# KAS-W/Deep-Reinforcement-Learning-Based-Signal-Gated-Market-Making

Hardware: AMD Instinct MI355X
Metric: env-steps/sec (pop×ticks) at 1/2/4/8 MI355X; generations/sec vs CPU ref (higher is better)
Workload: dtype f32+f64; 1 GPU; BASELINE config 3: 5 GA population(s) x 512 individuals (phi=0.0001 tick=0.001 510300, phi=0.001 tick=0.001 510300, phi=0.005 tick=0.001 510300, phi=0.008 tick=0.001 510300, phi=0.01 tick=0.001 510300), TradingPolicy 3->32->32->2, synthetic ticks (4560 train + 912 validation: the new master of each population), 1 GPU(s), weak scaling; config_id=3, populations=5, population_global=512, population_per_gpu=512, hidden=32, ticks_train=4560, ticks_val=912, adversary=False, val_mode=best, parallelism=population shards x1, hip_graph=True, walk_feedback=True

## Files before the change

deep-reinforcement-learning-based-signal-gated-market-making_amd/csrc/sgmm_frontier.hip:

```cpp
#include <cstddef>
#include <cstdlib>
#include <cstring>

#include "sgmm_mlp_mfma.h"

namespace sgmm {

#ifdef SGMM_STAMPS
constexpr int kStampWaves = 1 << 16;
__device__ unsigned long long g_tstamps[kStampWaves][8];
__device__ unsigned int g_thwid[kStampWaves][2];
#endif

struct FusedChain {
    double S;
    uint32_t st;
    int32_t tr;
};
template <class T>
__device__ __forceinline__ T fused_ld(const T* p) {
    typedef __attribute__((address_space(1))) const T gT;
    return __hip_atomic_load((gT*)p, __ATOMIC_RELAXED, __HIP_MEMORY_SCOPE_AGENT);
}
template <class T>
__device__ __forceinline__ void fused_st(T* p, T v) {
    typedef __attribute__((address_space(1))) T gT;
    __hip_atomic_store((gT*)p, v, __ATOMIC_RELAXED, __HIP_MEMORY_SCOPE_AGENT);
}

__device__ __forceinline__ FusedChain fused_group(const FrontierArgs& args, int e, int g, int CL, int nch,
                                                  FusedChain cs, double* win, uint32_t* kin, uint8_t* start) {
    const EpArrays& ep = args.ep;
    const int lane = (int)threadIdx.x;
    const int32_t T = ep.len[e];
    const int c0 = g * kFrontierLanes, c1 = min(nch, c0 + kFrontierLanes);
// ... 150 lines not shown
    if (ng > 1 && cg == 1) {
        if (threadIdx.x == 0) go = __hip_atomic_load(hs, __ATOMIC_RELAXED, __HIP_MEMORY_SCOPE_AGENT) == 1u;
        if (!__shfl(go, 0, kWave)) {
            fused_ship(args, e, CL, nch);
            if (threadIdx.x == 0) {
                asm volatile("s_waitcnt vmcnt(0)" ::: "memory");
                go = __hip_atomic_fetch_add(hs, 2u, __ATOMIC_RELAXED, __HIP_MEMORY_SCOPE_AGENT) == 1u;
            }
            if (!__shfl(go, 0, kWave)) return;
        }
        const double S0 = fused_ld(&ho->S);
        const uint32_t w = fused_ld(&ho->st_tr);
        cs = FusedChain{S0, w & 0xFFu, (int32_t)(w >> 8)};
        g = 1;
    }
    asm volatile("s_waitcnt vmcnt(0)" ::: "memory");
    for (;;) {
        cs = fused_group(args, e, g, CL, nch, cs, win, kin, start);
        if (g + 1 >= ng) break;
        go = 0;
        if (threadIdx.x == 0) {
            fused_st(&ho->S, cs.S);
            fused_st(&ho->st_tr, cs.st | ((uint32_t)cs.tr << 8));
            asm volatile("s_waitcnt vmcnt(0)" ::: "memory");
            go = __hip_atomic_fetch_add(hs, 1u, __ATOMIC_RELAXED, __HIP_MEMORY_SCOPE_AGENT) == 2u;
        }
        if (!__shfl(go, 0, kWave)) return;
        g = 1;
    }
    if (ng > 1 && threadIdx.x == 0) fused_st(hs, 0u);
    fused_finish(args, e, cs);
}

template <int H, int NSI, int LS, bool SP, bool FS = false>
__global__ __launch_bounds__(kWave) __attribute__((amdgpu_waves_per_eu(4))) void k_policy_frontier(FrontierArgs args) {
    static_assert(!FS || (LS == 1 && !SP), "the fused scan: one wave per walk, no spill");
    static_assert(H % 16 == 0 && H <= 32, "frontier kernel: H = 16 or 32");
    using L = GenomeLayout<H>;
    constexpr int NT = H / 16, KS = H / 4;
    constexpr int HP = 20;
    constexpr int kHb = kWave * HP * 4;
    constexpr int kBig = L::N * 4 > kHb ? L::N * 4 : kHb;
    __shared__ __attribute__((aligned(16))) unsigned char big[kBig];
    __shared__ __attribute__((aligned(16))) float w3i[2 * H + 2];
    __shared__ __attribute__((aligned(16))) float c1s[NT][4][4];
    __shared__ __attribute__((aligned(16))) float b2s[H];
    __shared__ __attribute__((aligned(8))) float sig[kWave][2];
    __shared__ double px[5][kWave];
    __shared__ uint16_t pl[kWave * (NSI - 1)];
    __shared__ uint32_t nslot_s;
    __shared__ uint32_t wid_s, tmin_s, t0_s, spk_s;
    constexpr int kFa0 = (int)(offsetof(FrontierArgs, ep) / 4), kFa1 = (int)(offsetof(FrontierArgs, src) / 4);
    constexpr int kFa2 = (int)(offsetof(FrontierArgs, inv_min) / 4), kFa3 = (int)(sizeof(FrontierArgs) / 4);
    constexpr int kFaWords = (kFa1 - kFa0) + (kFa3 - kFa2);
    static_assert(offsetof(FrontierArgs, src) % 4 == 0 && offsetof(FrontierArgs, inv_min) % 4 == 0 &&
                  sizeof(FrontierArgs) % 4 == 0, "whole words");
    __shared__ uint32_t fa_s[FS ? kFaWords : 1];
    __shared__ uint32_t ep_s, cl_s, nch_s, cg_s;
#if defined(__HIP_DEVICE_COMPILE__)
    if constexpr (FS) {
        typedef __attribute__((address_space(4))) const uint32_t ka_u32;
        const ka_u32* ka = (const ka_u32*)__builtin_amdgcn_kernarg_segment_ptr();
        for (int i = (int)threadIdx.x; i < kFaWords; i += kWave)
            fa_s[i] = ka[i < kFa1 - kFa0 ? kFa0 + i : kFa2 + i - (kFa1 - kFa0)];
    }
#endif
    if (SP && threadIdx.x == 0) {
        wid_s = blockIdx.x;
        spk_s = 0;
        t0_s = (uint32_t)wall_clock64();
        args.wspill[blockIdx.x] = 0u;
    }

    const sgmm_ticks& tk = args.tk;
    const EpArrays& ep = args.ep;
    const sgmm_env_params* __restrict__ params = args.params;
    const GenomeSrc& src = args.src;
    const int32_t inv_min = args.inv_min, nsi = args.nsi;
    uint64_t* __restrict__ cmaps = args.cmaps;
    uint32_t* __restrict__ ctr32 = args.ctr32;
    uint32_t* __restrict__ kinfo = args.kinfo;
    double* __restrict__ rew = args.rew;
    static_assert(LS == 1 || LS == 2 || LS == 4, "lane split 1, 2 or 4");
    constexpr int NL = kFrontierLanes / LS;
    int pos, cg, nw;
    frontier_wave(ep, (int)blockIdx.x / LS, pos, cg, nw);
    const int off = ((int)blockIdx.x % LS) * NL;
    const int e = ep.order ? ep.order[pos] : pos;
    const int32_t T = ep.len[e];
    if (T <= 0) {
        if (!FS || cg != 0) return;
        if (threadIdx.x == 0) {
            ep_s = (uint32_t)e;
            cl_s = 4u;
            nch_s = 0u;
            cg_s = 0u;
        }
    }
    if (T > 0) {
        const int CL = frontier_len(T, nw);
        const int nch = (T + CL - 1) / CL;
        if (cg * kFrontierLanes + off >= nch) return;
        if (FS && threadIdx.x == 0) {
            ep_s = (uint32_t)e;
            cl_s = (uint32_t)CL;
            nch_s = (uint32_t)nch;
            cg_s = (uint32_t)cg;
// ... 8 lines not shown

        float* gsm = reinterpret_cast<float*>(big);
        stage_genomes(src, e, ep.genome[e], -1, L::N, gsm, nullptr);
        __syncthreads();
        if (lane < 2 * H) w3i[lane] = gsm[L::W3 + (lane & 1) * H + (lane >> 1)];
        if (lane < 2) w3i[2 * H + lane] = gsm[L::B3 + lane];
        if (lane < H) {
            b2s[lane] = gsm[L::B2 + lane];
            c1s[lane >> 4][lane & 3][(lane >> 2) & 3] = gsm[L::B1 + lane];
        }
        float a1[NT];
#pragma unroll
        for (int hf = 0; hf < NT; ++hf)
            a1[hf] = grp < 3 ? gsm[L::W1 + 3 * (16 * hf + 4 * (col & 3) + (col >> 2)) + grp] : 0.0f;
        float w2f[NT][KS];
#pragma unroll
        for (int rt = 0; rt < NT; ++rt)
#pragma unroll
            for (int i = 0; i < KS; ++i) w2f[rt][i] = gsm[L::W2 + (16 * rt + col) * H + 4 * i + grp];
        __syncthreads();
        float* hb = reinterpret_cast<float*>(big);
        const sgmm_env_params p = params[ep.param[e]];

        const uint32_t all = (1u << nsi) - 1u;
        const uint32_t sset = (!lane_ok || c >= nch) ? 0u : (c == 0 ? 1u << (uint32_t)(-inv_min) : all);
        const uint32_t p0 = sset ? (uint32_t)__builtin_ctz(sset) : 0u;
        uint64_t cur = kIdentityMap;
        uint32_t cnt[(NSI + 1) / 2];
#pragma unroll
        for (int s = 0; s < (NSI + 1) / 2; ++s) cnt[s] = 0;
        uint32_t mcnt = 0;
        bool merged = __builtin_popcount(sset) <= 1;
        int kc = merged ? 0 : CL;
        auto tick_of = [&](int tt) { return tb + (ntl > 0 ? t0 : 0) + min(tt, max(ntl - 1, 0)); };
#ifdef SGMM_STAMPS
        unsigned long long lite_t0, lite_sl = 0, lite_ts = 0, lite_s8 = 0, lite_s16 = 0;
        asm volatile("s_memrealtime %0\n\ts_waitcnt lgkmcnt(0)" : "=s"(lite_t0)::"memory");
#endif
#ifdef SGMM_STAMPS_PHASE
        unsigned long long fs_t0, fs_a, fs_b, fs_c[7] = {0, 0, 0, 0, 0, 0, 0}, fs_r0;
#define SGMM_FT(var) asm volatile("s_memtime %0\n\ts_waitcnt lgkmcnt(0)" : "=s"(var)::"memory")
        asm volatile("s_memrealtime %0\n\ts_waitcnt lgkmcnt(0)" : "=s"(fs_r0)::"memory");
        SGMM_FT(fs_t0);
#define SGMM_PH(k)                    \
        do {                              \
            unsigned long long t_;        \
            SGMM_FT(t_);                  \
            fs_c[k] += t_ - fs_b;         \
            fs_b = t_;                    \
        } while (0)
#else
#define SGMM_PH(k) \
        do {           \
        } while (0)
#endif
        int64_t ti = tick_of(0);
        float ns1 = tk.s1n[ti], ns2 = tk.s2n[ti];
        int fr_extra = 0;
        if ((SP || LS == 1) && lane == 0) {
            nslot_s = 0;
            if (SP) tmin_s = (uint32_t)max(4, CL - kSpillTicks);
        }

        auto mlp = [&](auto nq, float& o0, float& o1, auto&& after_layer2) {
            constexpr int NQ = decltype(nq)::value;
            float xb[NQ];
#pragma unroll
            for (int q = 0; q < NQ; ++q) xb[q] = hb[(16 * q + col) * 4 + grp];
            f32x4 acc[NQ][NT];
#pragma unroll
            for (int q0 = 0; q0 < NQ; q0 += 2) {
                constexpr int Q2 = NQ < 2 ? NQ : 2;
                f32x4 h1[Q2][NT];
#pragma unroll
                for (int hf = 0; hf < NT; ++hf) {
                    const f32x4 cc = *reinterpret_cast<const f32x4*>(&c1s[hf][grp][0]);
#pragma unroll
                    for (int q = 0; q < Q2; ++q)
                        h1[q][hf] = __builtin_amdgcn_mfma_f32_16x16x4f32(a1[hf], xb[q0 + q], cc, 0, 0, 0);
                }
#pragma unroll
                for (int q = 0; q < Q2; ++q)
#pragma unroll
                    for (int hf = 0; hf < NT; ++hf)
#pragma unroll
                        for (int r = 0; r < 4; ++r) h1[q][hf][r] = relu(h1[q][hf][r]);
#pragma unroll
                for (int rt = 0; rt < NT; ++rt) {
                    const f32x4 bb = *reinterpret_cast<const f32x4*>(&b2s[16 * rt + 4 * grp]);
#pragma unroll
// ... 28 lines not shown
                    asm volatile("" : "+v"(w3p));
                    const f32x4 h = *reinterpret_cast<const f32x4*>(&hb[lane * HP + 4 * j4]);
#pragma unroll
                    for (int r2 = 0; r2 < 2; ++r2) {
                        const f32x4 w = *reinterpret_cast<lds_cf4*>(w3p + 4 * r2);
                        o0 = __builtin_fmaf(w[0], h[2 * r2], o0);
                        o1 = __builtin_fmaf(w[1], h[2 * r2], o1);
                        o0 = __builtin_fmaf(w[2], h[2 * r2 + 1], o0);
                        o1 = __builtin_fmaf(w[3], h[2 * r2 + 1], o1);
                    }
                }
                asm volatile("" ::: "memory");
            }
#ifdef SGMM_STAMPS_PHASE
            asm volatile("s_waitcnt vmcnt(0) lgkmcnt(0)" ::: "memory");
#endif
            SGMM_PH(2);
        };

#pragma unroll 1
        for (int tt = 0; tt < CL; ++tt) {
#ifdef SGMM_STAMPS_PHASE
            SGMM_FT(fs_b);
#endif
            if constexpr (SP) {
                if ((tt & 3) == 0 && (uint32_t)tt >= (uint32_t)__builtin_amdgcn_readfirstlane((int)tmin_s) &&
                    (uint32_t)wall_clock64() - (uint32_t)__builtin_amdgcn_readfirstlane((int)t0_s) > args.spill_budget) {
                    if (lane == 0) spk_s = (uint32_t)tt;
                    break;
                }
            }
            const bool act = tt < ntl;
            const float s1 = ns1, s2 = ns2;
            const int64_t tcur = ti;
            ti = tick_of(tt + 1);
            ns1 = tk.s1n[ti];
            ns2 = tk.s2n[ti];
            uint32_t fmask = 0;
            if (merged) {
                fmask = 1u << map_get(cur, p0);
            } else {
#pragma unroll
                for (int s = 0; s < NSI; ++s)
                    if ((sset >> s) & 1u) fmask |= 1u << map_get(cur, (uint32_t)s);
            }
            if (!act) fmask = 0;
            const uint32_t ext = fmask & (fmask - 1u);
            int epfx = 0, etot = 0;
            if (__ballot(ext != 0u)) {
                *reinterpret_cast<f32x2*>(&sig[lane][0]) = f32x2{s1, s2};
                const uint32_t nex = (uint32_t)__builtin_popcount(ext);
                const uint64_t eb0 = __ballot(nex & 1u), eb1 = __ballot(nex & 2u), eb2 = __ballot(nex & 4u);
                epfx = mbcnt64(eb0) + 2 * mbcnt64(eb1) + 4 * mbcnt64(eb2);
                etot = __popcll(eb0) + 2 * __popcll(eb1) + 4 * __popcll(eb2);
                uint32_t r = ext;
                int pp = epfx;
#pragma unroll
                for (int m = 0; m < NSI - 1; ++m)
                    if (r) {
                        pl[pp++] = (uint16_t)((lane << 3) | __builtin_ctz(r));
                        r &= r - 1u;
                    }
            }
            const bool any0 = __ballot(fmask != 0u) != 0ull;
            const int nx = (etot + kWave - 1) / kWave;
            fr_extra = fr_extra - (fr_extra >> 3) + (nx << 5);
            if ((SP || LS == 1) && lane == 0)
                __hip_atomic_fetch_add(&nslot_s, (uint32_t)((any0 ? 1 : 0) + nx), __ATOMIC_RELAXED, __HIP_MEMORY_SCOPE_WAVEFRONT);
            if ((tt & 7) == 7) {
                if (fr_extra > kFrPrioExtra) __builtin_amdgcn_s_setprio(2);
                else __builtin_amdgcn_s_setprio(0);
            }
#ifdef SGMM_STAMPS
            lite_sl += (any0 ? 1 : 0) + nx;
            if (tt == 7) lite_s8 = lite_sl;
            if (tt == 15) lite_s16 = lite_sl;
            lite_ts += (any0 ? 4 : 0) + (etot + 15) / 16;
#endif
            int64_t prs = ep.rs;
            asm volatile("" : "+s"(prs));
            const uint64_t pa = reinterpret_cast<uint64_t>(rew + rbase);
            uint64_t pu = ((uint64_t)(uint32_t)__builtin_amdgcn_readfirstlane((int)(uint32_t)(pa >> 32)) << 32) |
                          (uint32_t)__builtin_amdgcn_readfirstlane((int)(uint32_t)pa);
            asm volatile("" : "+s"(pu));
            double* const prow = reinterpret_cast<double*>(pu) + frontier_row(tt, off);
            uint64_t stepmap = kIdentityMap;
            uint32_t trm = 0;
#ifdef SGMM_STAMPS_PHASE
            fs_c[3] += (any0 ? 1 : 0) + nx;
            asm volatile("s_waitcnt vmcnt(0) lgkmcnt(0)" ::: "memory");
#endif
            SGMM_PH(5);
            if (any0) {
                const bool has = fmask != 0u;
                const uint32_t f = has ? (uint32_t)__builtin_ctz(fmask) : 0u;
                *reinterpret_cast<f32x4*>(&hb[lane * 4]) = f32x4{s1, s2, (float)(inv_min + (int)f) * 0.5f, 0.0f};
                float o0, o1;
                double tmid, task, tbid, tbmax, tsmin;
                mlp(IntC<NL / 16>{}, o0, o1, [&] {
                    tmid = tk.mid_next[tcur];
                    task = tk.best_ask[tcur];
                    tbid = tk.best_bid[tcur];
                    tbmax = tk.buy_max[tcur];
                    tsmin = tk.sell_min[tcur];
                });
                if (etot) {
                    px[0][lane] = tmid;
                    px[1][lane] = task;
                    px[2][lane] = tbid;
                    px[3][lane] = tbmax;
                    px[4][lane] = tsmin;
                }
                const int32_t oa = act_to_int(rintf(o0 * p.act_scale));
                const int32_t ob = act_to_int(rintf(o1 * p.act_scale));
                const StepOut so1 = ftp_step(p, inv_min + (int)f, oa, ob, tmid, task, tbid, tbmax, tsmin);
                if (has) {
                    const uint64_t to = (uint64_t)(f + so1.fill_buy - so1.fill_sell);
                    stepmap = (stepmap & ~(0xFFull << (8 * f))) | (to << (8 * f));
                    trm |= (uint32_t)(so1.fill_buy | so1.fill_sell) << f;
                    if (merged) {
                        prow[p0 * prs + lane] = so1.reward;
                    } else {
#pragma unroll
                        for (int s = 0; s < NSI; ++s)
                            if (((sset >> s) & 1u) && map_get(cur, (uint32_t)s) == f) prow[s * prs + lane] = so1.reward;
                    }
                }
#ifdef SGMM_STAMPS_PHASE
                asm volatile("s_waitcnt vmcnt(0) lgkmcnt(0)" ::: "memory");
#endif
                SGMM_PH(4);
            }
#pragma unroll 1
            for (int x = 0; x < nx; ++x) {
                const int pidx = kWave * x + lane;
                const bool has = pidx < etot;
                const uint32_t v = has ? (uint32_t)pl[pidx] : 0u;
// ... 277 lines not shown
                        const uint32_t ki = args.kinfo[ci];
                        const bool merged = (int)(ki & kKinfoTick) < CL;
                        const uint32_t p0 = ki >> 29;
                        const uint32_t all = (1u << nsi) - 1u;
                        const uint32_t sset = c == 0 ? 1u << (uint32_t)(-inv_min) : all;
                        const int sh = (lane >> shs) << shs;
                        const uint64_t segm = SEG == 64 ? ~0ull : (((1ull << SEG) - 1ull) << sh);
                        const int ntl = has ? min(T, (c + 1) * CL) - c * CL : 0;
                        const bool last = valid && u == ntl - K - 1;
                        uint64_t cm = cur;
#pragma unroll
                        for (int st = 0; st < NSI; ++st) {
                            const bool tr = st < nsi && ((sset >> st) & 1u);
                            const uint32_t x = map_get(cur, (uint32_t)st);
                            const uint32_t y = map_get(excl, x & 7u);
                            if (valid && tr && (!merged || (uint32_t)st == p0))
                                args.rew[(int64_t)st * ep.rs + rbase + frontier_row(K + u, lg)] = rl_s[y & 7u][lane];
                            const uint32_t cnt = (uint32_t)__popcll(__ballot(valid && tr && ((traded >> (y & 7u)) & 1u)) & segm);
                            if (last && tr) {
                                args.ctr32[ci * 8 + st] += cnt;
                                cm = (cm & ~(0xFFull << (8 * st))) | ((uint64_t)map_get(inc, x & 7u) << (8 * st));
                            }
                        }
                        if (last) args.cmaps[ci] = cm;
                    }
                    __syncthreads();
                }
            }
            __syncthreads();
        }
    }
}

int launch_frontier_spill(int hidden, int nsi, unsigned n_waves, int ls, hipStream_t s, const FrontierArgs& fa) {
    if (!fa.spill_budget || !fa.wspill || n_waves == 0) return SGMM_OK;
    const int total = (int)(n_waves * (unsigned)ls);
    const dim3 grid(kSpillBlocks), block(kWave * nsi);
    with_int<16, 32>(hidden, [&](auto h) {
        with_int<5, 8>(nsi <= 5 ? 5 : 8, [&](auto n) {
            SGMM_LAUNCH((k_frontier_spill<decltype(h)::value, decltype(n)::value>), grid, block, 0, s, fa, total, ls);
        });
    });
    SGMM_LAUNCHED();
    return SGMM_OK;
}

int launch_policy_frontier(int hidden, int nsi, unsigned n_waves, int ls, hipStream_t s, const FrontierArgs& fa) {
    const dim3 grid(n_waves), block(kWave);
    if (fa.fitness && (ls != 1 || fa.ep.ngrp > kFusedMaxGroups || fa.spill_budget || !fa.handoff || !fa.hstate)) {
        set_error("fused path scan: one wave per walk, <= %d groups, no spill, hand-off arrays", kFusedMaxGroups);
        return SGMM_ERR_ARG;
    }
    with_int<16, 32>(hidden, [&](auto h) {
        with_int<5, 8>(nsi <= 5 ? 5 : 8, [&](auto n) {
            constexpr int H = decltype(h)::value, NSI = decltype(n)::value;
            if (fa.fitness) {
                SGMM_LAUNCH((k_policy_frontier<H, NSI, 1, false, true>), grid, block, 0, s, fa);
                return;
            }
            with_bool(fa.spill_budget && fa.wspill, [&](auto sp) {
                with_int<4, 2, 1>(ls, [&](auto l) {
                    SGMM_LAUNCH((k_policy_frontier<H, NSI, decltype(l)::value, decltype(sp)::value>),
                                dim3(n_waves * (unsigned)ls), block, 0, s, fa);
                });
            });
        });
// ... 16 lines not shown
```

deep-reinforcement-learning-based-signal-gated-market-making_amd/csrc/sgmm_plan.h:

```cpp
#pragma once

#include <algorithm>
#include <cstddef>
#include <cstdint>

#include "../../include/sgmm.h"

#if defined(__HIPCC__)
#define SGMM_PLAN_HD __host__ __device__ __forceinline__
#else
#define SGMM_PLAN_HD inline
#endif

namespace sgmm {

constexpr int kWave = 64;
constexpr int kChunk = 64;
constexpr int kScanBlock = 256;
constexpr int kMaxLen = 1 << 17;
constexpr int kFrontierLanes = 64;
constexpr int kFrontierMaxWaves = 16;
constexpr int64_t kFrontierMaxLen = (int64_t)kFrontierLanes * 65532;
constexpr int kFusedMaxGroups = 2;
constexpr int kFusedHandoffBytes = 16;
constexpr int kScanThreads = 1024;
constexpr int kScanAt1024 = 256;
constexpr int kScanAt512 = 512;
constexpr int kScanArlAt1024 = 1024;
#ifndef SGMM_LANES_W
#define SGMM_LANES_W 4
#endif
constexpr int kLanesW = SGMM_LANES_W;
constexpr int kReorderMaxPops = 64;

SGMM_PLAN_HD int frontier_len(int T, int nw) {
    const int c = (T + kFrontierLanes * nw - 1) / (kFrontierLanes * nw);
    return c < 4 ? 4 : (c + 3) & ~3;
}
SGMM_PLAN_HD int64_t frontier_pad(int nw) { return 256LL * nw + 16; }

struct PlanKnobs {
    int32_t policy_path = -1;
    int32_t groups = -1;
    int32_t lane_split = -1;
    int32_t tail = -1;
    int32_t four = -1;
    int32_t min_eps = -1;
    int32_t table_sp = -1;
    int32_t scan_threads = -1;
    int32_t reorder_weights = -1;
    int32_t spill = -1;
    int32_t seq_sum = -1;
    int32_t fused_scan = -1;
    int32_t lanes_scan = -1;
};
static_assert(sizeof(PlanKnobs) == SGMM_PLAN_N * sizeof(int32_t), "one field per SGMM_PLAN_* knob");

struct LaunchShape {
    int32_t n = 0;
    int32_t max_len = 0;
    int64_t total_steps = 0;
    int32_t nsi = 0;
    int32_t hidden = 0;
    bool arl = false;
    int32_t simds = 0;
    bool tail = false;
    int32_t mode = 0;
    int32_t pop_eps = 0;
    int32_t src_pop_eps = 0;
    bool walk_feedback = false;
};

constexpr size_t kNoSection = ~size_t(0);
struct WorkspaceLayout {
    size_t cmaps = kNoSection, ctr = kNoSection, kinfo = kNoSection, wslots = kNoSection, wspill = kNoSection,
           arrive = kNoSection, handoff = kNoSection, fills = kNoSection, rew = kNoSection;
    int64_t rs = 0;
    size_t bytes = 0;
};

struct FrontierPlan {
    int32_t g0, gtail, whole, gmax;
    int64_t waves;
    int32_t ls;
};

enum class PolicyKernel { Frontier, TableSp, TableV3, TableMfma, TableValu };
enum class ScanKernel { Fused, Lanes, Wave, Arl };

struct LaunchPlan {
    PolicyKernel policy;
    FrontierPlan fr;
    uint32_t spill;
    ScanKernel scan;
    int32_t scan_threads;
    int32_t scan_grid;
    int32_t seq_sum;
    int32_t lanes_w;
    bool validation;
    bool reorder;
    uint32_t w_whole, w_split;
    WorkspaceLayout ws;
};

constexpr int kFrontierAutoWaves = 8;
inline FrontierPlan frontier_plan(int32_t n, int32_t simds, const PlanKnobs& k) {
    FrontierPlan p{1, 1, std::max(n, 0), 1, std::max<int64_t>(n, 0), 1};
    const int ls_force = k.lane_split;
    if (ls_force == 2 || ls_force == 4) p.ls = ls_force;
    {
        const int g = k.groups;
// ... 17 lines not shown
    } else if (tail && four && p.g0 == 1 && 2 * n - 4 * S >= S / 2 && n < 4 * S) {
        p.whole = (int32_t)(2 * n - 4 * S);
        p.gtail = p.gmax = 2;
    } else if (tail && p.g0 == 1 && n > S && r > 0) {
        const int64_t gt = std::max<int64_t>(1, std::min<int64_t>(kFrontierMaxWaves, (S + r / 2) / r));
        if (gt > 1) {
            p.whole = (int32_t)(n - r);
            p.gtail = p.gmax = (int32_t)gt;
        }
    }
    p.waves = (int64_t)p.whole * p.g0 + (int64_t)(n - p.whole) * p.gtail;
    return p;
}

inline int64_t plane_stride(int64_t steps, int32_t n, bool arl, int32_t gmax) {
    const int64_t pad = arl ? 0 : frontier_pad(gmax) * n;
    return (steps + pad + 31) & ~int64_t(31);
}

inline WorkspaceLayout workspace_layout(int32_t n, int64_t total_steps, int32_t nsi, bool arl, int32_t gmax) {
    WorkspaceLayout L;
    L.rs = plane_stride(total_steps, n, arl, gmax);
    if (total_steps < 0 || nsi <= 0 || nsi > 8 || n < 0) return L;
    size_t at = 0;
    const auto section = [&at](size_t bytes) {
        const size_t off = at;
        at += (bytes + 255) & ~size_t(255);
        return off;
    };
    const size_t steps = (size_t)total_steps, ne = (size_t)n;
    if (arl) {
        L.fills = section(steps * sizeof(uint64_t));
        L.rew = at;
        L.bytes = at + (size_t)L.rs * (size_t)(4 * nsi) * sizeof(double);
        return L;
    }
    const size_t slots = steps / kChunk + ne + 1;
    const size_t recs = ne * kFrontierLanes * (size_t)gmax;
    L.cmaps = section(std::max(slots, recs) * sizeof(uint64_t));
    L.ctr = section(std::max(slots * sizeof(uint64_t), recs * 8 * sizeof(uint32_t)));
    L.kinfo = section(recs * sizeof(uint32_t));
    L.wslots = section(ne * 64 * sizeof(uint32_t));
    L.wspill = section(ne * 64 * sizeof(uint32_t));
    L.arrive = section(ne * sizeof(uint32_t));
    L.handoff = section(ne * kFusedHandoffBytes);
    L.rew = at;
    L.bytes = at + (size_t)L.rs * (size_t)nsi * sizeof(double);
    return L;
}
inline WorkspaceLayout workspace_layout(int32_t n, int64_t total_steps, int32_t nsi, bool arl, int32_t simds,
                                        const PlanKnobs& k) {
    return workspace_layout(n, total_steps, nsi, arl, frontier_plan(n, simds, k).gmax);
}

constexpr int kFrontierMinEps = 512;
constexpr int64_t kTableSpChunks = 256;
inline PolicyKernel policy_kernel(const LaunchShape& sh, const PlanKnobs& k) {
    const bool h1632 = sh.hidden == 16 || sh.hidden == 32;
    const int path = k.policy_path;
    if (!sh.arl && h1632) {
        if (sh.max_len > kMaxLen || path == 1) return PolicyKernel::Frontier;
        if (path <= 0 && sh.n >= (k.min_eps > 0 ? k.min_eps : kFrontierMinEps)) return PolicyKernel::Frontier;
    }
    if (sh.hidden == 8 || path == 3) return PolicyKernel::TableValu;
    if (sh.arl || !h1632) return PolicyKernel::TableMfma;
    const int64_t nch = (sh.max_len + kChunk - 1) / kChunk;
    const bool sp = k.table_sp >= 0 ? k.table_sp != 0 : nch * sh.n <= kTableSpChunks;
    return sp ? PolicyKernel::TableSp : PolicyKernel::TableV3;
}

inline LaunchPlan resolve_plan(const LaunchShape& sh, const PlanKnobs& k) {
    LaunchPlan p{};
    p.policy = policy_kernel(sh, k);
    p.fr = frontier_plan(sh.n, sh.simds, k);
    p.ws = workspace_layout(sh.n, sh.total_steps, sh.nsi, sh.arl, p.fr.gmax);
    const bool fr = p.policy == PolicyKernel::Frontier;
    p.validation = sh.tail && (sh.mode == 2 || sh.mode == 4);
    const bool plain_tail = !sh.tail || sh.mode == 3;

    if (fr && k.spill > 0 && sh.max_len > 0) p.spill = (uint32_t)std::min<int64_t>((int64_t)k.spill * 100, 0x7FFFFFFF);

    const int P = sh.src_pop_eps;
    p.reorder = fr && sh.tail && sh.mode == 3 && sh.walk_feedback && P > 0 && sh.n % P == 0 && sh.n / P >= 2 &&
                sh.n / P <= kReorderMaxPops && p.fr.ls == 1 && p.fr.g0 == 1 && (p.fr.gtail == 2 || p.fr.gtail == 4) &&
                p.fr.whole > 0 && p.fr.whole < sh.n && sh.total_steps == (int64_t)sh.n * sh.max_len;
    p.w_whole = 5;
    p.w_split = 4;
    if (const int w = k.reorder_weights; w > 0 && (w >> 8) > 0 && (w & 255) > 0) {
        p.w_whole = (uint32_t)(w >> 8) & 63u;
        p.w_split = (uint32_t)w & 63u;
    }

    if (fr && sh.max_len > 0 && k.fused_scan != 0 && !p.validation && !p.spill && p.fr.ls == 1 &&
        p.fr.gmax <= kFusedMaxGroups && k.seq_sum != 0 && plain_tail && (k.fused_scan == 1 || p.fr.gmax == 1)) {
        p.scan = ScanKernel::Fused;
        return p;
    }

    const auto seq_sum = [&](int nt) {
        if (k.seq_sum >= 0) return k.seq_sum != 0;
        return p.validation || (!sh.arl && nt <= 256);
    };
    p.scan_grid = sh.n;
    if (sh.arl) {
        p.scan = ScanKernel::Arl;
        p.scan_threads = sh.n <= kScanArlAt1024 ? kScanThreads : kScanBlock;
        p.seq_sum = seq_sum(p.scan_threads);
        return p;
// ... 23 lines not shown
```

deep-reinforcement-learning-based-signal-gated-market-making_amd/csrc/sgmm_rollout.h:

```cpp
#pragma once

#include "sgmm_device.h"
#include "sgmm_ga_device.h"
#include "sgmm_internal.h"
#include "sgmm_plan.h"

namespace sgmm {

constexpr int kSeg = 4096;

struct EpArrays {
    const int32_t* genome;
    const int32_t* adv;
    const int64_t* tick_off;
    const int32_t* len;
    const int64_t* step_off;
    const int32_t* param;
    int64_t rs;
    const int32_t* order;
    int32_t ngrp;
    int32_t g0, gtail, whole;
    int32_t seq_sum = 0;
};

// ... 120 lines not shown
    }
}
constexpr uint32_t kKinfoTick = 0xFFFFu;
__host__ __device__ __forceinline__ uint32_t kinfo_groups(uint32_t k) { return (k >> 20) & 31u; }

struct StepArgs {
    sgmm_ga_state* st;
    float* master_mm;
    float* master_adv;
    float* best_master;
    int64_t n_mm, n_adv;
    uint64_t seed;
    sgmm_ga_history* history;
    int32_t hist_cap;
    int32_t P;
    int32_t pop_eps;
    const uint64_t* seeds;
    int32_t mode;
};

__device__ __forceinline__ void store_record(double* fitness, int32_t* trades, int e, double f,
                                             int32_t t) {
    typedef __attribute__((address_space(1))) double gdouble;
    typedef __attribute__((address_space(1))) int32_t gint;
    __hip_atomic_store((gdouble*)(fitness + e), f, __ATOMIC_RELAXED, __HIP_MEMORY_SCOPE_AGENT);
    __hip_atomic_store((gint*)(trades + e), t, __ATOMIC_RELAXED, __HIP_MEMORY_SCOPE_AGENT);
}

struct FrontierArgs {
    sgmm_ticks tk;
    EpArrays ep;
    const sgmm_env_params* params;
    GenomeSrc src;
    int32_t inv_min, nsi;
    uint64_t* cmaps;
    uint32_t* ctr32;
    uint32_t* kinfo;
    double* rew;
    uint32_t* wslots;
    uint32_t* wspill;
    uint32_t spill_budget;
    double* fitness;
    int32_t* trades;
    struct FusedHandoff* handoff;
    uint32_t* hstate;
    int32_t n_eps;
    StepArgs step;
};
struct FusedHandoff {
    double S;
    uint32_t st_tr;
    uint32_t pad;
};
static_assert(sizeof(FusedHandoff) == kFusedHandoffBytes, "the workspace layout's hand-off size");
constexpr int kFusedWin = 512;
constexpr int kSpillTicks = 64;

template <int SEG>
__device__ __forceinline__ uint64_t wave_map_scan_seg(uint64_t m) {
#define SGMM_MSTEP(CTRL, RM) m = map_then(dpp64<CTRL, RM>(kIdentityMap, m), m);
    SGMM_MSTEP(0x111, 0xF) SGMM_MSTEP(0x112, 0xF) SGMM_MSTEP(0x114, 0xF) SGMM_MSTEP(0x118, 0xF)
    if constexpr (SEG >= 32) { SGMM_MSTEP(0x142, 0xA) }
    if constexpr (SEG >= 64) { SGMM_MSTEP(0x143, 0xC) }
#undef SGMM_MSTEP
    return m;
}

int launch_policy_frontier(int hidden, int nsi, unsigned n_waves, int ls, hipStream_t s, const FrontierArgs& fa);
int launch_frontier_spill(int hidden, int nsi, unsigned n_waves, int ls, hipStream_t s, const FrontierArgs& fa);

struct ReorderJob {
    const uint32_t* wslots;
    int32_t* order;
    int32_t n, whole, gtail, pop_eps;
    uint32_t w_whole = 5, w_split = 4;
    int32_t len = 0;
};
void launch_policy_table(PolicyKernel kind, int hidden, bool arl, int nsi, int max_len, int n_ep,
                         const sgmm_ticks& tk, const EpArrays& ep, const sgmm_env_params* params,
                         const GenomeSrc& src, int32_t inv_min, uint64_t* ctr, uint64_t* cmaps, uint64_t* fills,
                         double* rew, const ReorderJob* rj, hipStream_t s);
void launch_walk_reorder(const ReorderJob& job, hipStream_t s);

}
```

deep-reinforcement-learning-based-signal-gated-market-making_amd/csrc/sgmm_rollout.hip:

```cpp
#include <algorithm>
#include <climits>
#include <atomic>
#include <cstdlib>
#include <cstdio>
#include <cstring>

#include "sgmm_rollout.h"

namespace sgmm {

__device__ __forceinline__ int next_state_arl(int s, int code) {
    const int fb = code & 1, fs = code >> 1;
    return (((s >> 2) + fb - fs) << 2) | (fs << 1) | fb;
}
__device__ __forceinline__ int arl_step(int s, uint64_t f, int& cnt) {
    const int c = (int)(f >> (2 * s)) & 3;
    cnt += c != 0;
    const int d = __builtin_amdgcn_sbfe(0x00FC0400, 8 * c, 8);
    return ((s + d) & ~3) | c;
}

#ifdef SGMM_STAMPS
__device__ unsigned long long g_stamps[4096][16];
#define SGMM_STAMP(e, k)                                                           \
// ... 1129 lines not shown
    if (hipGetDevice(&dev) != hipSuccess || dev < 0) dev = 0;
    std::atomic<int>& c = cache[dev < kMaxDev ? dev : kMaxDev - 1];
    int n = c.load(std::memory_order_relaxed);
    if (n == 0) {
        int cus = 0;
        if (hipDeviceGetAttribute(&cus, hipDeviceAttributeMultiprocessorCount, dev) != hipSuccess || cus <= 0)
            cus = 256;
        n = 4 * cus;
        c.store(n, std::memory_order_relaxed);
    }
    return n;
}

static EpArrays ep_arrays(const sgmm_episodes* e, bool with_adv, int64_t rs) {
    return EpArrays{e->genome, with_adv ? e->adv : nullptr, e->tick_off, e->len, e->step_off,
                    e->param, rs, e->order, 1, 1, 1, e->n};
}

}

using namespace sgmm;

#ifdef SGMM_STAMPS
extern "C" int sgmm_debug_stamps(unsigned long long* host, int n_eps) {
    return (int)hipMemcpyFromSymbol(host, HIP_SYMBOL(g_stamps), sizeof(unsigned long long) * 16 * n_eps);
}
extern "C" int sgmm_debug_tail(unsigned long long* host) {
    return (int)hipMemcpyFromSymbol(host, HIP_SYMBOL(g_tail), sizeof(unsigned long long) * 8);
}
#endif

static size_t rollout_ws_bytes(int32_t n_episodes, int64_t total_steps, int32_t nsi, bool arl,
                               const PlanKnobs& knobs) {
    return workspace_layout(n_episodes, total_steps, nsi, arl, simd_count(), knobs).bytes;
}

extern "C" size_t sgmm_rollout_workspace_bytes(int32_t n_episodes, int64_t total_steps, int32_t n_inventory,
                                               int32_t with_adversary) {
    return rollout_ws_bytes(n_episodes, total_steps, n_inventory, with_adversary != 0, plan_knobs());
}

extern "C" size_t sgmm_rollout_workspace_size(int32_t n_episodes, int64_t total_steps,
                                              int32_t n_states) {
    if (n_states > 8) return n_states % 4 ? 0 : rollout_ws_bytes(n_episodes, total_steps, n_states / 4, true, plan_knobs());
    return rollout_ws_bytes(n_episodes, total_steps, n_states, false, plan_knobs());
}

extern "C" int sgmm_ordered_sum(const double* values, int64_t n, double init, double* out,
                                void* stream) {
    clear_error();
    SGMM_REQUIRE(out && (values || n == 0) && n >= 0, "bad arguments");
    ProfScope prof("ordered_sum", as_stream(stream));
    SGMM_LAUNCH(k_ordered_sum, dim3(1), dim3(kScanThreads), 0, as_stream(stream), values, n,
                       init, out);
    SGMM_LAUNCHED();
    return SGMM_OK;
}


template <int NSM, bool FR>
static void launch_path_scan(int nt, int64_t n, size_t lds, hipStream_t s, const EpArrays& ep,
                             const sgmm_env_params* params, int32_t inv_min, const uint64_t* cmaps,
                             const uint64_t* ctr, const uint32_t* kinfo, const double* rew, double* fitness,
                             int32_t* trades, const StepArgs& step) {
    if (nt == kWave)
        SGMM_LAUNCH((k_path_scan<NSM, 4 * kWave, FR, kWave>), dim3(n), dim3(nt), lds, s, ep, params, inv_min, cmaps,
                    ctr, kinfo, rew, fitness, trades, step);
// ... 10 lines not shown


__global__ __launch_bounds__(1024) void k_zero_u32(uint32_t* __restrict__ p, int32_t n) {
    const int i = (int)(blockIdx.x * blockDim.x + threadIdx.x);
    if (i < n) p[i] = 0u;
}


static int rollout_impl(const PlanKnobs& knobs, const sgmm_ticks* ticks, const sgmm_episodes* eps,
                        const sgmm_env_params* params, const GenomeSrc& src, bool arl,
                        int32_t hidden, double* fitness, int32_t* trades, void* workspace,
                        size_t workspace_bytes, const StepArgs& step, hipStream_t s,
                        ReorderJob* rj_out = nullptr, const ReorderJob* rj_in = nullptr,
                        int32_t* walk_order = nullptr) {
    SGMM_REQUIRE(fitness && trades, "null fitness/trades output");
    if (eps->n == 0) return SGMM_OK;
    const int32_t nsi = eps->inv_max - eps->inv_min + 1;
    const int32_t ns = arl ? 4 * nsi : nsi;
    LaunchShape shape;
    shape.n = eps->n;
    shape.max_len = eps->max_len;
    shape.total_steps = eps->total_steps;
    shape.nsi = nsi;
    shape.hidden = hidden;
    shape.arl = arl;
    shape.simds = simd_count();
    shape.tail = step.st != nullptr;
    shape.mode = step.mode;
    shape.pop_eps = step.pop_eps;
    shape.src_pop_eps = src.pop_eps;
    shape.walk_feedback = walk_order && eps->order == walk_order;
    const LaunchPlan plan = resolve_plan(shape, knobs);
    const WorkspaceLayout& ws = plan.ws;
    if (!workspace || workspace_bytes < ws.bytes) {
        set_error("workspace %zu bytes < required %zu", workspace_bytes, ws.bytes);
        return SGMM_ERR_WORKSPACE;
    }
    char* w = reinterpret_cast<char*>(workspace);
    const auto at = [w](size_t off) -> void* { return off == kNoSection ? nullptr : w + off; };
    uint64_t* cmaps = static_cast<uint64_t*>(at(ws.cmaps));
    uint64_t* ctr = static_cast<uint64_t*>(at(ws.ctr));
    uint32_t* kinfo = static_cast<uint32_t*>(at(ws.kinfo));
    uint32_t* wslots = static_cast<uint32_t*>(at(ws.wslots));
    uint32_t* wspill = static_cast<uint32_t*>(at(ws.wspill));
    uint32_t* arrive = static_cast<uint32_t*>(at(ws.arrive));
    FusedHandoff* handoff = static_cast<FusedHandoff*>(at(ws.handoff));
    uint64_t* fills = static_cast<uint64_t*>(at(ws.fills));
    double* rew = static_cast<double*>(at(ws.rew));
    EpArrays ep = ep_arrays(eps, arl, ws.rs);
    const bool fr = plan.policy == PolicyKernel::Frontier;
    if (fr) {
        ep.ngrp = plan.fr.gmax;
        ep.g0 = plan.fr.g0;
        ep.gtail = plan.fr.gtail;
        ep.whole = plan.fr.whole;
    }
    const bool vt = plan.validation;
    SGMM_REQUIRE(fr || arl || eps->max_len <= kMaxLen,
                 "max_len=%d > %d needs the frontier kernel (hidden 16 or 32) or the adversary path", eps->max_len,
                 kMaxLen);
    SGMM_REQUIRE(!fr || eps->max_len <= kFrontierMaxLen, "max_len=%d > %lld ticks per episode",
                 eps->max_len, (long long)kFrontierMaxLen);
    const ReorderJob* rj_fold = nullptr;
    if (rj_in && rj_in->order) {
        if (plan.policy == PolicyKernel::TableSp && eps->max_len > 0 &&
            reinterpret_cast<const char*>(rj_in->wslots) >= w + ws.bytes) {
            rj_fold = rj_in;
        } else {
            launch_walk_reorder(*rj_in, s);
            SGMM_LAUNCHED();
        }
    }
    if (eps->max_len <= 0) {
    } else if (fr) {
        FrontierArgs fa{*ticks, ep, params, src, eps->inv_min, nsi, cmaps, reinterpret_cast<uint32_t*>(ctr),
                        kinfo, rew, wslots, wspill, plan.spill};
        if (plan.scan == ScanKernel::Fused) {
            fa.fitness = fitness;
            fa.trades = trades;
            fa.hstate = arrive;
            fa.handoff = handoff;
            fa.n_eps = eps->n;
            fa.step = step;
            if (plan.fr.gmax > 1)
                SGMM_LAUNCH(k_zero_u32, dim3((eps->n + 1023) / 1024), dim3(1024), 0, s, arrive, eps->n);
        }
        ProfScope prof(vt ? "val_policy_frontier" : "policy_frontier", s);
        if (int rc = launch_policy_frontier(hidden, nsi, (unsigned)plan.fr.waves, plan.fr.ls, s, fa)) return rc;
        if (fa.spill_budget) {
            ProfScope prof2(vt ? "val_frontier_spill" : "frontier_spill", s);
            if (int rc = launch_frontier_spill(hidden, nsi, (unsigned)plan.fr.waves, plan.fr.ls, s, fa)) return rc;
        }
    } else {
        ProfScope prof(vt ? "val_policy_table" : "policy_table", s);
        launch_policy_table(plan.policy, hidden, arl, nsi, eps->max_len, eps->n, *ticks, ep, params, src,
                            eps->inv_min, ctr, cmaps, fills, rew, rj_fold, s);
        SGMM_LAUNCHED();
    }
    if (plan.scan != ScanKernel::Fused) {
        ProfScope prof(vt ? "val_path_scan" : "path_scan", s);
        const int nt = plan.scan_threads;
        const dim3 grid(plan.scan_grid), block(nt);
        ep.seq_sum = plan.seq_sum;
        if (plan.scan == ScanKernel::Arl) {
            size_t lds = arl_scan_lds(ns);
            if (step.st) lds = std::max(lds, step_lds_bytes(nt, step));
            if (nt == kScanThreads)
                SGMM_LAUNCH(k_path_scan_arl<kScanThreads>, grid, block, lds, s, ep, params, eps->inv_min,
                            nsi, fills, rew, fitness, trades, step);
// ... 336 lines not shown
```

Before: 25.00 billion env-steps/s.

## Pre-gather per-population tick columns into lane-coalesced views for the frontier kernel

Adds a k_tick_views pre-pass that gathers each population's tick columns (s1n, s2n, mid, ask, bid, buy_max, sell_min) into a workspace region laid out per chunk-group, tick and lane. Each lane's per-tick loads in the frontier kernel become contiguous across the wave instead of strided by chunk length. Tick-table pointers are read from the kernarg segment and kept scalar through readfirstlane, with 32-bit offsets in place of 64-bit indexing. The cost is an extra kernel launch, a larger workspace, and duplicated tick data per population and group.

```diff
diff --git a/deep-reinforcement-learning-based-signal-gated-market-making_amd/csrc/sgmm_frontier.hip b/deep-reinforcement-learning-based-signal-gated-market-making_amd/csrc/sgmm_frontier.hip
--- a/deep-reinforcement-learning-based-signal-gated-market-making_amd/csrc/sgmm_frontier.hip
+++ b/deep-reinforcement-learning-based-signal-gated-market-making_amd/csrc/sgmm_frontier.hip
@@ -1,6 +1,7 @@
 #include <cstddef>
 #include <cstdlib>
 #include <cstring>
+#include <type_traits>
 
 #include "sgmm_mlp_mfma.h"
 
@@ -217,6 +218,8 @@
     fused_finish(args, e, cs);
 }
 
+static_assert(std::is_trivially_copyable_v<FrontierArgs> && std::is_standard_layout_v<FrontierArgs>,
+              "FrontierArgs is read back word by word from the kernarg segment");
 template <int H, int NSI, int LS, bool SP, bool FS = false>
 __global__ __launch_bounds__(kWave) __attribute__((amdgpu_waves_per_eu(4))) void k_policy_frontier(FrontierArgs args) {
     static_assert(!FS || (LS == 1 && !SP), "the fused scan: one wave per walk, no spill");
@@ -257,7 +260,6 @@
         args.wspill[blockIdx.x] = 0u;
     }
 
-    const sgmm_ticks& tk = args.tk;
     const EpArrays& ep = args.ep;
     const sgmm_env_params* __restrict__ params = args.params;
     const GenomeSrc& src = args.src;
@@ -332,7 +334,41 @@
         uint32_t mcnt = 0;
         bool merged = __builtin_popcount(sset) <= 1;
         int kc = merged ? 0 : CL;
-        auto tick_of = [&](int tt) { return tb + (ntl > 0 ? t0 : 0) + min(tt, max(ntl - 1, 0)); };
+        typedef __attribute__((address_space(4))) const sgmm_ticks tick_table;
+        uint64_t ptab = 0;
+#if defined(__HIP_DEVICE_COMPILE__)
+        ptab = (uint64_t)__builtin_amdgcn_kernarg_segment_ptr() + offsetof(FrontierArgs, tk);
+#endif
+        int64_t ub = tb;
+        uint32_t loff = ntl > 0 ? (uint32_t)t0 : 0u;
+        int ts = 1;
+        if (args.views) {
+            const int vk = src.pop_eps > 0 ? e / src.pop_eps : 0;
+            if (vk < kTickViewPops) {
+                const TickViewHeader* vh = reinterpret_cast<const TickViewHeader*>(args.views) + 2 * vk + (nw == ep.g0 ? 0 : 1);
+                if (vh->valid && vh->tb == tb && vh->T == T) {
+                    ptab = reinterpret_cast<uint64_t>(&vh->cols);
+                    ub = 0;
+                    loff = (uint32_t)tick_view_entry(cg, 0, off + lane, CL);
+                    ts = kFrontierLanes;
+                }
+            }
+        }
+        ts = __builtin_amdgcn_readfirstlane(ts);
+        ptab = ((uint64_t)(uint32_t)__builtin_amdgcn_readfirstlane((int)(uint32_t)(ptab >> 32)) << 32) |
+               (uint32_t)__builtin_amdgcn_readfirstlane((int)(uint32_t)ptab);
+        auto table = [&] {
+            uint64_t q = ptab;
+            asm volatile("" : "+s"(q));
+            return reinterpret_cast<tick_table*>(q);
+        };
+        ub = (int64_t)(((uint64_t)(uint32_t)__builtin_amdgcn_readfirstlane((int)(uint32_t)((uint64_t)ub >> 32)) << 32) |
+                       (uint32_t)__builtin_amdgcn_readfirstlane((int)(uint32_t)ub));
+        auto tick_of = [&](int tt) { return loff + (uint32_t)(min(tt, max(ntl - 1, 0)) * ts); };
+        auto col_at = [&](auto* colp, uint32_t i) {
+            using V = std::remove_pointer_t<decltype(colp)>;
+            return *reinterpret_cast<V*>(reinterpret_cast<const char*>(colp + ub) + (uint32_t)(i * (uint32_t)sizeof(V)));
+        };
 #ifdef SGMM_STAMPS
         unsigned long long lite_t0, lite_sl = 0, lite_ts = 0, lite_s8 = 0, lite_s16 = 0;
         asm volatile("s_memrealtime %0\n\ts_waitcnt lgkmcnt(0)" : "=s"(lite_t0)::"memory");
@@ -354,8 +390,13 @@
         do {           \
         } while (0)
 #endif
-        int64_t ti = tick_of(0);
-        float ns1 = tk.s1n[ti], ns2 = tk.s2n[ti];
+        float ns1, ns2;
+        {
+            tick_table* t = table();
+            const uint32_t ti = tick_of(0);
+            ns1 = col_at(t->s1n, ti);
+            ns2 = col_at(t->s2n, ti);
+        }
         int fr_extra = 0;
         if ((SP || LS == 1) && lane == 0) {
             nslot_s = 0;
@@ -450,10 +491,12 @@
             }
             const bool act = tt < ntl;
             const float s1 = ns1, s2 = ns2;
-            const int64_t tcur = ti;
-            ti = tick_of(tt + 1);
-            ns1 = tk.s1n[ti];
-            ns2 = tk.s2n[ti];
+            {
+                tick_table* t = table();
+                const uint32_t ti = tick_of(tt + 1);
+                ns1 = col_at(t->s1n, ti);
+                ns2 = col_at(t->s2n, ti);
+            }
             uint32_t fmask = 0;
             if (merged) {
                 fmask = 1u << map_get(cur, p0);
@@ -516,11 +559,13 @@
                 float o0, o1;
                 double tmid, task, tbid, tbmax, tsmin;
                 mlp(IntC<NL / 16>{}, o0, o1, [&] {
-                    tmid = tk.mid_next[tcur];
-                    task = tk.best_ask[tcur];
-                    tbid = tk.best_bid[tcur];
-                    tbmax = tk.buy_max[tcur];
-                    tsmin = tk.sell_min[tcur];
+                    tick_table* t = table();
+                    const uint32_t tcur = tick_of(tt);
+                    tmid = col_at(t->mid_next, tcur);
+                    task = col_at(t->best_ask, tcur);
+                    tbid = col_at(t->best_bid, tcur);
+                    tbmax = col_at(t->buy_max, tcur);
+                    tsmin = col_at(t->sell_min, tcur);
                 });
                 if (etot) {
                     px[0][lane] = tmid;
@@ -864,6 +909,42 @@
     }
 }
 
+constexpr int kTickViewBlocks = 32, kTickViewThreads = 256;
+__global__ __launch_bounds__(kTickViewThreads) void k_tick_views(sgmm_ticks tk, const int64_t* __restrict__ tick_off,
+                                                                const int32_t* __restrict__ len, int32_t n,
+                                                                int32_t pop_eps, int32_t g0, int32_t gtail,
+                                                                int32_t whole, unsigned char* views, uint32_t cap) {
+    const int slot = (int)blockIdx.y, k = slot >> 1, w = slot & 1;
+    const int64_t e = pop_eps > 0 ? (int64_t)k * pop_eps : (k == 0 ? 0 : n);
+    const bool want = e < n && (w == 0 ? whole > 0 : (whole < n && gtail != g0));
+    const int g = w ? gtail : g0;
+    const int32_t T = want ? len[e] : 0;
+    const int64_t tb = want ? tick_off[e] : 0;
+    const int64_t entries = T > 0 ? tick_view_entries(T, g) : 0;
+    const bool valid = T > 0 && entries <= (int64_t)cap;
+    const sgmm_ticks v = tick_view_columns(views, slot, cap);
+    if (blockIdx.x == 0 && threadIdx.x == 0)
+        reinterpret_cast<TickViewHeader*>(views)[slot] = TickViewHeader{tb, T, valid ? 1 : 0, v, {}};
+    if (!valid) return;
+    for (uint32_t i = blockIdx.x * kTickViewThreads + threadIdx.x; i < (uint32_t)entries;
+         i += kTickViewBlocks * kTickViewThreads) {
+        const int64_t t = tb + tick_view_source(T, g, i);
+        const_cast<float*>(v.s1n)[i] = tk.s1n[t];
+        const_cast<float*>(v.s2n)[i] = tk.s2n[t];
+        const_cast<double*>(v.mid_next)[i] = tk.mid_next[t];
+        const_cast<double*>(v.best_ask)[i] = tk.best_ask[t];
+        const_cast<double*>(v.best_bid)[i] = tk.best_bid[t];
+        const_cast<double*>(v.buy_max)[i] = tk.buy_max[t];
+        const_cast<double*>(v.sell_min)[i] = tk.sell_min[t];
+    }
+}
+
+void launch_tick_views(int32_t n_eps, hipStream_t s, const FrontierArgs& fa) {
+    SGMM_LAUNCH(k_tick_views, dim3(kTickViewBlocks, kTickViewSlots), dim3(kTickViewThreads), 0, s, fa.tk,
+                fa.ep.tick_off, fa.ep.len, n_eps, fa.src.pop_eps, fa.ep.g0, fa.ep.gtail, fa.ep.whole,
+                const_cast<unsigned char*>(fa.views), fa.view_cap);
+}
+
 int launch_frontier_spill(int hidden, int nsi, unsigned n_waves, int ls, hipStream_t s, const FrontierArgs& fa) {
     if (!fa.spill_budget || !fa.wspill || n_waves == 0) return SGMM_OK;
     const int total = (int)(n_waves * (unsigned)ls);
diff --git a/deep-reinforcement-learning-based-signal-gated-market-making_amd/csrc/sgmm_plan.h b/deep-reinforcement-learning-based-signal-gated-market-making_amd/csrc/sgmm_plan.h
--- a/deep-reinforcement-learning-based-signal-gated-market-making_amd/csrc/sgmm_plan.h
+++ b/deep-reinforcement-learning-based-signal-gated-market-making_amd/csrc/sgmm_plan.h
@@ -39,6 +39,26 @@
 }
 SGMM_PLAN_HD int64_t frontier_pad(int nw) { return 256LL * nw + 16; }
 
+constexpr int kTickViewPops = 8;
+constexpr int kTickViewSlots = 2 * kTickViewPops;
+constexpr int kTickViewSlotHeader = 128;
+constexpr int kTickViewHeader = kTickViewSlots * kTickViewSlotHeader;
+constexpr int kTickViewEntryBytes = 5 * 8 + 2 * 4;
+SGMM_PLAN_HD int64_t tick_view_entries(int T, int g) { return (int64_t)g * frontier_len(T, g) * kFrontierLanes; }
+SGMM_PLAN_HD int64_t tick_view_entry(int cg, int tt, int l, int CL) {
+    return ((int64_t)cg * CL + tt) * kFrontierLanes + l;
+}
+SGMM_PLAN_HD int64_t tick_view_source(int T, int g, int64_t entry) {
+    const uint32_t CL = (uint32_t)frontier_len(T, g);
+    const uint32_t l = (uint32_t)entry % kFrontierLanes, row = (uint32_t)entry / kFrontierLanes;
+    const uint32_t cg = row / CL, tt = row - cg * CL;
+    const uint32_t t0 = (cg * kFrontierLanes + l) * CL;
+    const uint32_t end = t0 + CL < (uint32_t)T ? t0 + CL : (uint32_t)T;
+    const uint32_t ntl = end > t0 ? end - t0 : 0u;
+    const uint32_t last = ntl > 0 ? ntl - 1 : 0u;
+    return (int64_t)((ntl > 0 ? t0 : 0u) + (tt < last ? tt : last));
+}
+
 struct PlanKnobs {
     int32_t policy_path = -1;
     int32_t groups = -1;
@@ -77,6 +97,9 @@
            arrive = kNoSection, handoff = kNoSection, fills = kNoSection, rew = kNoSection;
     int64_t rs = 0;
     size_t bytes = 0;
+    size_t views = kNoSection;
+    int64_t view_cap = 0;
+    size_t total = 0;
 };
 
 struct FrontierPlan {
@@ -160,7 +183,7 @@
     if (arl) {
         L.fills = section(steps * sizeof(uint64_t));
         L.rew = at;
-        L.bytes = at + (size_t)L.rs * (size_t)(4 * nsi) * sizeof(double);
+        L.bytes = L.total = at + (size_t)L.rs * (size_t)(4 * nsi) * sizeof(double);
         return L;
     }
     const size_t slots = steps / kChunk + ne + 1;
@@ -173,15 +196,27 @@
     L.arrive = section(ne * sizeof(uint32_t));
     L.handoff = section(ne * kFusedHandoffBytes);
     L.rew = at;
-    L.bytes = at + (size_t)L.rs * (size_t)nsi * sizeof(double);
+    L.bytes = L.total = at + (size_t)L.rs * (size_t)nsi * sizeof(double);
     return L;
+}
+constexpr int kFrontierMinEps = 512;
+inline void add_tick_views(WorkspaceLayout& L, int32_t n, int64_t total_steps, bool arl, int32_t gmax,
+                           const PlanKnobs& k) {
+    if (L.bytes == 0 || arl || n <= 0 || total_steps <= 0) return;
+    if (!(k.policy_path == 1 || (k.policy_path <= 0 && n >= (k.min_eps > 0 ? k.min_eps : kFrontierMinEps)))) return;
+    const int64_t mean = (total_steps + n - 1) / n;
+    L.view_cap = (mean + 256LL * gmax + kFrontierLanes - 1) & ~int64_t(kFrontierLanes - 1);
+    L.views = (L.bytes + 255) & ~size_t(255);
+    L.total = L.views + kTickViewHeader + (size_t)kTickViewSlots * (size_t)L.view_cap * kTickViewEntryBytes;
 }
 inline WorkspaceLayout workspace_layout(int32_t n, int64_t total_steps, int32_t nsi, bool arl, int32_t simds,
                                         const PlanKnobs& k) {
-    return workspace_layout(n, total_steps, nsi, arl, frontier_plan(n, simds, k).gmax);
-}
-
-constexpr int kFrontierMinEps = 512;
+    const int32_t gmax = frontier_plan(n, simds, k).gmax;
+    WorkspaceLayout L = workspace_layout(n, total_steps, nsi, arl, gmax);
+    add_tick_views(L, n, total_steps, arl, gmax, k);
+    return L;
+}
+
 constexpr int64_t kTableSpChunks = 256;
 inline PolicyKernel policy_kernel(const LaunchShape& sh, const PlanKnobs& k) {
     const bool h1632 = sh.hidden == 16 || sh.hidden == 32;
@@ -202,6 +237,7 @@
     p.policy = policy_kernel(sh, k);
     p.fr = frontier_plan(sh.n, sh.simds, k);
     p.ws = workspace_layout(sh.n, sh.total_steps, sh.nsi, sh.arl, p.fr.gmax);
+    add_tick_views(p.ws, sh.n, sh.total_steps, sh.arl, p.fr.gmax, k);
     const bool fr = p.policy == PolicyKernel::Frontier;
     p.validation = sh.tail && (sh.mode == 2 || sh.mode == 4);
     const bool plain_tail = !sh.tail || sh.mode == 3;
diff --git a/deep-reinforcement-learning-based-signal-gated-market-making_amd/csrc/sgmm_rollout.h b/deep-reinforcement-learning-based-signal-gated-market-making_amd/csrc/sgmm_rollout.h
--- a/deep-reinforcement-learning-based-signal-gated-market-making_amd/csrc/sgmm_rollout.h
+++ b/deep-reinforcement-learning-based-signal-gated-market-making_amd/csrc/sgmm_rollout.h
@@ -176,6 +176,7 @@
     EpArrays ep;
     const sgmm_env_params* params;
     GenomeSrc src;
+    const unsigned char* views;
     int32_t inv_min, nsi;
     uint64_t* cmaps;
     uint32_t* ctr32;
@@ -184,6 +185,7 @@
     uint32_t* wslots;
     uint32_t* wspill;
     uint32_t spill_budget;
+    uint32_t view_cap;
     double* fitness;
     int32_t* trades;
     struct FusedHandoff* handoff;
@@ -191,6 +193,20 @@
     int32_t n_eps;
     StepArgs step;
 };
+struct TickViewHeader {
+    int64_t tb;
+    int32_t T;
+    int32_t valid;
+    sgmm_ticks cols;
+    uint64_t pad_[7];
+};
+static_assert(sizeof(TickViewHeader) == kTickViewSlotHeader, "the region's header block");
+__host__ __device__ __forceinline__ sgmm_ticks tick_view_columns(const unsigned char* views, int slot, uint32_t cap) {
+    const unsigned char* b = views + kTickViewHeader + (size_t)slot * cap * kTickViewEntryBytes;
+    const double* d = reinterpret_cast<const double*>(b);
+    const float* f = reinterpret_cast<const float*>(d + (size_t)5 * cap);
+    return sgmm_ticks{f, f + cap, d, d + cap, d + (size_t)2 * cap, d + (size_t)3 * cap, d + (size_t)4 * cap};
+}
 struct FusedHandoff {
     double S;
     uint32_t st_tr;
@@ -212,6 +228,7 @@
 
 int launch_policy_frontier(int hidden, int nsi, unsigned n_waves, int ls, hipStream_t s, const FrontierArgs& fa);
 int launch_frontier_spill(int hidden, int nsi, unsigned n_waves, int ls, hipStream_t s, const FrontierArgs& fa);
+void launch_tick_views(int32_t n_eps, hipStream_t s, const FrontierArgs& fa);
 
 struct ReorderJob {
     const uint32_t* wslots;
diff --git a/deep-reinforcement-learning-based-signal-gated-market-making_amd/csrc/sgmm_rollout.hip b/deep-reinforcement-learning-based-signal-gated-market-making_amd/csrc/sgmm_rollout.hip
--- a/deep-reinforcement-learning-based-signal-gated-market-making_amd/csrc/sgmm_rollout.hip
+++ b/deep-reinforcement-learning-based-signal-gated-market-making_amd/csrc/sgmm_rollout.hip
@@ -1185,7 +1185,7 @@
 
 static size_t rollout_ws_bytes(int32_t n_episodes, int64_t total_steps, int32_t nsi, bool arl,
                                const PlanKnobs& knobs) {
-    return workspace_layout(n_episodes, total_steps, nsi, arl, simd_count(), knobs).bytes;
+    return workspace_layout(n_episodes, total_steps, nsi, arl, simd_count(), knobs).total;
 }
 
 extern "C" size_t sgmm_rollout_workspace_bytes(int32_t n_episodes, int64_t total_steps, int32_t n_inventory,
@@ -1262,8 +1262,8 @@
     shape.walk_feedback = walk_order && eps->order == walk_order;
     const LaunchPlan plan = resolve_plan(shape, knobs);
     const WorkspaceLayout& ws = plan.ws;
-    if (!workspace || workspace_bytes < ws.bytes) {
-        set_error("workspace %zu bytes < required %zu", workspace_bytes, ws.bytes);
+    if (!workspace || workspace_bytes < ws.total) {
+        set_error("workspace %zu bytes < required %zu", workspace_bytes, ws.total);
         return SGMM_ERR_WORKSPACE;
     }
     char* w = reinterpret_cast<char*>(workspace);
@@ -1294,7 +1294,7 @@
     const ReorderJob* rj_fold = nullptr;
     if (rj_in && rj_in->order) {
         if (plan.policy == PolicyKernel::TableSp && eps->max_len > 0 &&
-            reinterpret_cast<const char*>(rj_in->wslots) >= w + ws.bytes) {
+            reinterpret_cast<const char*>(rj_in->wslots) >= w + ws.total) {
             rj_fold = rj_in;
         } else {
             launch_walk_reorder(*rj_in, s);
@@ -1303,8 +1303,14 @@
     }
     if (eps->max_len <= 0) {
     } else if (fr) {
-        FrontierArgs fa{*ticks, ep, params, src, eps->inv_min, nsi, cmaps, reinterpret_cast<uint32_t*>(ctr),
-                        kinfo, rew, wslots, wspill, plan.spill};
+        FrontierArgs fa{*ticks, ep, params, src, static_cast<const unsigned char*>(at(ws.views)), eps->inv_min, nsi,
+                        cmaps, reinterpret_cast<uint32_t*>(ctr), kinfo, rew, wslots, wspill, plan.spill,
+                        (uint32_t)ws.view_cap};
+        if (fa.views) {
+            ProfScope prof(vt ? "val_tick_views" : "tick_views", s);
+            launch_tick_views(eps->n, s, fa);
+            SGMM_LAUNCHED();
+        }
         if (plan.scan == ScanKernel::Fused) {
             fa.fitness = fitness;
             fa.trades = trades;
```

New measurement: 25.11 billion env-steps/s, median of 6. No clear change (+0.4%).
